# Zhangwenyao1/DreamVLA

Measured on AMD Instinct MI355X. Metric: train samples/sec (CALVIN ABC->D, seq_len=7), higher is better.
Workload: dtype bf16; 1 GPU; DreamVLA CALVIN finetune step, head set C (obs_pred+depth_pred+sam_feat_pred+use_dit_head), B=32/GPU, S=7, window 10, 2x224^2 views, 77 text tokens, hidden 1024 / 24 layers / 16 heads, dropout 0.1 on, AdamW + clip 0.1; global_batch=32, seq_len=7, parallelism=dp1, grad_exchange=GradBucketReducer (flat bf16 buckets, async all-reduce), optimizer=FlatAdamW (HIP: dvla_sumsq_bf16 + dvla_adamw_bf16 on flat buffers)

## Files before the change

### dreamvla_amd/csrc/attention.hip

```cpp
#include "common.h"
#include "launch.h"
#include "../../include/dvla.h"

namespace {

constexpr int AT_THREADS = 256;
constexpr int RM72 = 72;
constexpr int RM_BYTES = 32 * RM72 * 2;
constexpr int PI_BYTES = 16 * 64 * 4;
constexpr float LOG2E = 1.4426950408889634f;
constexpr float LN2 = 0.6931471805599453f;

struct AttnKArgs {
  const bf16_t *q, *k, *v; bf16_t* o;
  int64_t qsb, qst, qsh, ksb, kst, ksh, vsb, vst, vsh, osb, ost, osh;
  int B, H, Lq, Lk;
  float scale;
  const int32_t* key_index;
  const uint32_t *bits_q, *bits_k;
  const uint8_t* tile_map; int nqt, nkt;
  int has_drop; uint32_t drop_thr; float inv_keep; uint32_t seed_lo, seed_hi;
  float c1;
  float* lse;
  const bf16_t* dout; int64_t dsb, dst, dsh;
// ... 856 lines not shown
      const int qq = qt0 * 32 + ql;
      bits[i] = qq < p.Lq ? p.bits_q[(int64_t)qq * p.nkt + kt] : 0u;
    }
  uint32_t rowkey = 0;
  if (p.has_drop) rowkey = drop_rowkey(p.seed_lo, p.seed_hi, (uint32_t)rowid);
  f32x16 dqacc[2] = {zero16(), zero16()};
  __syncthreads();
  const TileWords tw = tile_words(flags, p.nkt, wave, lane);

  auto next_needed = [&](int kt) -> int {
    if (tw.n) return tw.next(kt);
    while (kt < p.nkt && __builtin_amdgcn_readfirstlane((int)flags[kt]) == 0) ++kt;
    return kt < p.nkt ? kt : -1;
  };
  const uint32_t smem_base = (uint32_t)(uintptr_t)(__attribute__((address_space(3))) char*)smem;
  const int rl = 8 * wave + (lane >> 3);
  const int oct = (lane & 7) ^ fa_sw(rl);
  const uint32_t kst2 = (uint32_t)p.kst * 2u, vst2 = (uint32_t)p.vst * 2u;
  auto issue = [&](int kt, int slot) {
    int row = kt * 32 + rl;
    row = row < p.Lk ? row : p.Lk - 1;
    const uint32_t src = p.key_index ? (uint32_t)kidx[row] : (uint32_t)row;
    const uint32_t dst = smem_base + (uint32_t)(slot * FA_STAGE + wave * 1024);
    fa_glds16(kb, src * kst2 + oct * 16, __builtin_amdgcn_readfirstlane(dst));
    fa_glds16(vb, src * vst2 + oct * 16, __builtin_amdgcn_readfirstlane(dst + FA_TILE));
  };

  int kt = next_needed(0);
  int kti = kt, islot = 0, cslot = 0, inflight = 0;
#pragma unroll
  for (int d = 0; d < FA_NS - 1; ++d)
    if (kti >= 0) {
      issue(kti, islot);
      islot = (islot + 1) & (FA_NS - 1); ++inflight;
      kti = next_needed(kti + 1);
    }
#pragma unroll
  for (int s = 0; s < 4; ++s) { fa_settle(qf[s]); fa_settle(dof[s]); }
  fa_settle(lse2); fa_settle(dlt);
  while (kt >= 0) {
    if (inflight >= 3) fa_wait_vmcnt<4>();
    else if (inflight == 2) fa_wait_vmcnt<2>();
    else fa_wait_vmcnt<0>();
    __builtin_amdgcn_s_barrier();
    __builtin_amdgcn_sched_barrier(0);
    --inflight;
    if (kti >= 0) {
      issue(kti, islot);
      islot = (islot + 1) & (FA_NS - 1); ++inflight;
      kti = next_needed(kti + 1);
    }
    __builtin_amdgcn_sched_barrier(0);
    const int flag = tw.n ? tw.flag(kt) : (__builtin_amdgcn_readfirstlane((int)flags[kt]) >> (2 * wave)) & 3;
    if (flag != 0) {
      const char* ks = smem + cslot * FA_STAGE;
      const char* vs = ks + FA_TILE;
      f32x16 sacc = zero16(), dpacc = zero16();
      {
        bf16x8 fk[4], fv[4];
#pragma unroll
        for (int s = 0; s < 4; ++s) { fk[s] = fa_frag_rm(ks, l31, s, g); fv[s] = fa_frag_rm(vs, l31, s, g); }
        fa_group4(fk); fa_group4(fv);
#pragma unroll
        for (int s = 0; s < 4; ++s) {
          sacc = __builtin_amdgcn_mfma_f32_32x32x16_bf16(fk[s], qf[s], sacc, 0, 0, 0);
          dpacc = __builtin_amdgcn_mfma_f32_32x32x16_bf16(fv[s], dof[s], dpacc, 0, 0, 0);
        }
      }
      const int k0 = kt * 32;
      uint32_t vis = 0xffffffffu;
      if (flag == 2) vis = bits[(wave * 32 + l31) * p.nkt + kt];
      if (k0 + 32 > p.Lk) vis &= low_mask(p.Lk - k0);
      float ds[16];
#pragma unroll
      for (int r = 0; r < 16; ++r) ds[r] = fast_exp2(fmaf(sacc[r], scale_log2, -lse2));
      if (__any(vis != 0xffffffffu)) {
        const uint32_t vg = vis >> (4 * g);
        vis_select16<0u>(vg, ds);
      }
      if (p.has_drop) {
        const uint32_t tk = drop_tilekey(rowkey, (uint32_t)kt);
        const uint32_t dx = drop_rot(tk, (uint32_t)g);
#pragma unroll
        for (int r = 0; r < 16; ++r) {
          const float dp = (drop_elem(dx, tk, DVLA_DROP_C(r)) >= p.drop_thr) ? dpacc[r] : 0.f;
          ds[r] = ds[r] * fmaf(dp, c1, -dlt);
        }
      } else {
#pragma unroll
        for (int r = 0; r < 16; ++r) ds[r] = ds[r] * fmaf(dpacc[r], c1, -dlt);
      }
      const bf16x8 f0 = pack_frag(ds), f1 = pack_frag(ds + 8);
      bf16x8 kt4[4];
#pragma unroll
      for (int i = 0; i < 4; ++i) kt4[i] = fa_frag_tr(ks, i >> 1, i & 1, lane);
      fa_group4(kt4);
      dqacc[0] = __builtin_amdgcn_mfma_f32_32x32x16_bf16(kt4[0], f0, dqacc[0], 0, 0, 0);
      dqacc[1] = __builtin_amdgcn_mfma_f32_32x32x16_bf16(kt4[2], f0, dqacc[1], 0, 0, 0);
      dqacc[0] = __builtin_amdgcn_mfma_f32_32x32x16_bf16(kt4[1], f1, dqacc[0], 0, 0, 0);
      dqacc[1] = __builtin_amdgcn_mfma_f32_32x32x16_bf16(kt4[3], f1, dqacc[1], 0, 0, 0);
    }
    __builtin_amdgcn_sched_barrier(0);
    cslot = (cslot + 1) & (FA_NS - 1);
    kt = next_needed(kt + 1);
  }
  if (q_ok) store_token(p.dq + (int64_t)b * p.dqsb + (int64_t)q * p.dqst + (int64_t)h * p.dqsh, dqacc, 1.0f, g, (p.st16 & 2) != 0);
}

__host__ __device__ inline size_t fa_dkv_smem_bytes(int nqt, bool has_bits, bool has_drop) {
  return (size_t)FA_RING + fa_pad16(nqt) + (has_bits ? (size_t)128 * nqt * 4 : 0) + (size_t)2 * 32 * nqt * 4 +
         (has_drop ? (size_t)4 * 32 * nqt * 4 : 0);
}

__global__ __launch_bounds__(AT_THREADS) void attn_bwd_dkv_ring_kernel(AttnKArgs p) {
  extern __shared__ __attribute__((aligned(16))) char smem[];
  const int t = threadIdx.x, lane = t & 63, l31 = lane & 31, g = lane >> 5;
  const int wave = __builtin_amdgcn_readfirstlane(t >> 6);
  const int b = blockIdx.z, h = blockIdx.y;
  const int kt0 = blockIdx.x * 4;
  const int ktw = kt0 + wave;
  const int key = ktw * 32 + l31;
  const bool key_ok = key < p.Lk;
  const int key_row = (key_ok && p.key_index) ? p.key_index[key] : key;
  const float scale_log2 = p.scale * LOG2E;
  const float c1 = p.c1;
  const bool has_bits = p.tile_map != nullptr && p.bits_k != nullptr;
  const bf16_t* qb = p.q + (int64_t)b * p.qsb + (int64_t)h * p.qsh;
  const bf16_t* kb = p.k + (int64_t)b * p.ksb + (int64_t)h * p.ksh;
  const bf16_t* vb = p.v + (int64_t)b * p.vsb + (int64_t)h * p.vsh;
  const bf16_t* dob = p.dout + (int64_t)b * p.dsb + (int64_t)h * p.dsh;
  const int bh_row0 = (b * p.H + h) * p.Lq;

  uint8_t* flags = reinterpret_cast<uint8_t*>(smem + FA_RING);
  uint32_t* bits = reinterpret_cast<uint32_t*>(smem + FA_RING + fa_pad16(p.nqt));
  float* lse2s = reinterpret_cast<float*>(smem + FA_RING + fa_pad16(p.nqt) + (has_bits ? (size_t)128 * p.nqt * 4 : 0));
  float* dlts = lse2s + 32 * p.nqt;
  uint32_t* tks = reinterpret_cast<uint32_t*>(dlts + 32 * p.nqt);

  bf16x8 kf[4], vf[4];
#pragma unroll
  for (int s = 0; s < 4; ++s) {
    const uint4 a = load16(kb + (int64_t)key_row * p.kst + 16 * s + 8 * g, key_ok);
    const uint4 c = load16(vb + (int64_t)key_row * p.vst + 16 * s + 8 * g, key_ok);
    kf[s] = *reinterpret_cast<const bf16x8*>(&a);
    vf[s] = *reinterpret_cast<const bf16x8*>(&c);
  }
  for (int qt = t; qt < p.nqt; qt += AT_THREADS) {
    int f = 0;
#pragma unroll
    for (int w = 0; w < 4; ++w) f |= tile_flag(p, qt, kt0 + w) << (2 * w);
    flags[qt] = (uint8_t)f;
  }
  if (has_bits)
    for (int i = t; i < 128 * p.nqt; i += AT_THREADS) {
      const int kl = i / p.nqt, qt = i - kl * p.nqt;
      const int kk = kt0 * 32 + kl;
      bits[i] = kk < p.Lk ? p.bits_k[(int64_t)kk * p.nqt + qt] : 0u;
    }
  for (int i = t; i < 32 * p.nqt; i += AT_THREADS) {
    lse2s[i] = i < p.Lq ? p.lse[bh_row0 + i] * LOG2E : INFINITY;
    dlts[i] = i < p.Lq ? p.delta[bh_row0 + i] * p.scale : 0.f;
    if (p.has_drop) {
      const uint32_t rk = drop_rowkey(p.seed_lo, p.seed_hi, (uint32_t)(bh_row0 + i));
#pragma unroll
      for (int w = 0; w < 4; ++w) tks[w * 32 * p.nqt + i] = drop_tilekey(rk, (uint32_t)(kt0 + w));
    }
  }
  const uint32_t drop_cj = DVLA_DROP_C((l31 & 3) + 4 * (l31 >> 3));
  const uint32_t drop_half = (uint32_t)((l31 >> 2) & 1);
  const uint32_t* tkw = tks + wave * 32 * p.nqt;
  f32x16 dkacc[2] = {zero16(), zero16()}, dvacc[2] = {zero16(), zero16()};
  __syncthreads();
  const TileWords tw = tile_words(flags, p.nqt, wave, lane);

  auto next_needed = [&](int qt) -> int {
    if (tw.n) return tw.next(qt);
    while (qt < p.nqt && __builtin_amdgcn_readfirstlane((int)flags[qt]) == 0) ++qt;
    return qt < p.nqt ? qt : -1;
  };
  const uint32_t smem_base = (uint32_t)(uintptr_t)(__attribute__((address_space(3))) char*)smem;
  const int rl = 8 * wave + (lane >> 3);
  const int oct = (lane & 7) ^ fa_sw(rl);
  const uint32_t qst2 = (uint32_t)p.qst * 2u, dst2 = (uint32_t)p.dst * 2u;
  auto issue = [&](int qt, int slot) {
    int row = qt * 32 + rl;
    row = row < p.Lq ? row : p.Lq - 1;
    const uint32_t dst = smem_base + (uint32_t)(slot * FA_STAGE + wave * 1024);
    fa_glds16(qb, (uint32_t)row * qst2 + oct * 16, __builtin_amdgcn_readfirstlane(dst));
    fa_glds16(dob, (uint32_t)row * dst2 + oct * 16, __builtin_amdgcn_readfirstlane(dst + FA_TILE));
  };

  int qt = next_needed(0);
  int qti = qt, islot = 0, cslot = 0, inflight = 0;
#pragma unroll
  for (int d = 0; d < FA_NS - 1; ++d)
    if (qti >= 0) {
      issue(qti, islot);
      islot = (islot + 1) & (FA_NS - 1); ++inflight;
      qti = next_needed(qti + 1);
    }
#pragma unroll
  for (int s = 0; s < 4; ++s) { fa_settle(kf[s]); fa_settle(vf[s]); }
  while (qt >= 0) {
    asm volatile("" : "+a"(dkacc[0]), "+a"(dkacc[1]), "+a"(dvacc[0]), "+a"(dvacc[1]));
    if (inflight >= 3) fa_wait_vmcnt<4>();
    else if (inflight == 2) fa_wait_vmcnt<2>();
    else fa_wait_vmcnt<0>();
    __builtin_amdgcn_s_barrier();
    __builtin_amdgcn_sched_barrier(0);
    --inflight;
    if (qti >= 0) {
      issue(qti, islot);
      islot = (islot + 1) & (FA_NS - 1); ++inflight;
      qti = next_needed(qti + 1);
    }
    __builtin_amdgcn_sched_barrier(0);
    const int flag = tw.n ? tw.flag(qt) : (__builtin_amdgcn_readfirstlane((int)flags[qt]) >> (2 * wave)) & 3;
    if (flag != 0) {
      const char* qs = smem + cslot * FA_STAGE;
      const char* dos = qs + FA_TILE;
      f32x16 sacc = zero16(), dpacc = zero16();
      {
        bf16x8 fq[4], fd[4];
#pragma unroll
        for (int s = 0; s < 4; ++s) { fq[s] = fa_frag_rm(qs, l31, s, g); fd[s] = fa_frag_rm(dos, l31, s, g); }
        fa_group4(fq); fa_group4(fd);
#pragma unroll
        for (int s = 0; s < 4; ++s) {
          sacc = __builtin_amdgcn_mfma_f32_32x32x16_bf16(fq[s], kf[s], sacc, 0, 0, 0);
          dpacc = __builtin_amdgcn_mfma_f32_32x32x16_bf16(fd[s], vf[s], dpacc, 0, 0, 0);
        }
      }
      asm volatile("" : "+v"(sacc), "+v"(dpacc));
      const int q0 = qt * 32;
      float lse2[16], dlt[16];
#pragma unroll
      for (int rq = 0; rq < 4; ++rq) {
        const float4 a = *reinterpret_cast<const float4*>(lse2s + q0 + 8 * rq + 4 * g);
        const float4 c = *reinterpret_cast<const float4*>(dlts + q0 + 8 * rq + 4 * g);
        lse2[4 * rq] = a.x; lse2[4 * rq + 1] = a.y; lse2[4 * rq + 2] = a.z; lse2[4 * rq + 3] = a.w;
        dlt[4 * rq] = c.x; dlt[4 * rq + 1] = c.y; dlt[4 * rq + 2] = c.z; dlt[4 * rq + 3] = c.w;
      }
      uint32_t vis = key_ok ? 0xffffffffu : 0u;
      if (flag == 2) vis = bits[(wave * 32 + l31) * p.nqt + qt];
      float pr[16], ds[16];
#pragma unroll
      for (int r = 0; r < 16; ++r) pr[r] = fast_exp2(fmaf(sacc[r], scale_log2, -lse2[r]));
      if (__any(vis != 0xffffffffu)) {
        const uint32_t vg = vis >> (4 * g);
        vis_select16<0u>(vg, pr);
      }
      float dp[16];
#pragma unroll
      for (int r = 0; r < 16; ++r) dp[r] = dpacc[r];
#pragma unroll
      for (int r = 0; r < 16; ++r) ds[r] = pr[r];
      if (p.has_drop) {
#pragma unroll
        for (int rq = 0; rq < 4; ++rq) {
          const uint4 a = *reinterpret_cast<const uint4*>(tkw + q0 + 8 * rq + 4 * g);
          const uint32_t rk[4] = {a.x, a.y, a.z, a.w};
#pragma unroll
          for (int e = 0; e < 4; ++e) {
            const int r = 4 * rq + e;
            const bool keep = drop_elem(drop_rot(rk[e], drop_half), rk[e], drop_cj) >= p.drop_thr;
            dp[r] = keep ? dp[r] : 0.f;
            pr[r] = keep ? pr[r] : 0.f;
          }
        }
      }
#pragma unroll
      for (int r = 0; r < 16; ++r) ds[r] = ds[r] * fmaf(dp[r], c1, -dlt[r]);
      const bf16x8 pf0 = pack_frag(pr), pf1 = pack_frag(pr + 8);
      const bf16x8 sf0 = pack_frag(ds), sf1 = pack_frag(ds + 8);
      {
        bf16x8 td[4], tq[4];
#pragma unroll
        for (int i = 0; i < 4; ++i) { td[i] = fa_frag_tr(dos, i >> 1, i & 1, lane); tq[i] = fa_frag_tr(qs, i >> 1, i & 1, lane); }
        fa_group4(td); fa_group4(tq);
        dvacc[0] = __builtin_amdgcn_mfma_f32_32x32x16_bf16(td[0], pf0, dvacc[0], 0, 0, 0);
        dkacc[0] = __builtin_amdgcn_mfma_f32_32x32x16_bf16(tq[0], sf0, dkacc[0], 0, 0, 0);
        dvacc[1] = __builtin_amdgcn_mfma_f32_32x32x16_bf16(td[2], pf0, dvacc[1], 0, 0, 0);
        dkacc[1] = __builtin_amdgcn_mfma_f32_32x32x16_bf16(tq[2], sf0, dkacc[1], 0, 0, 0);
        dvacc[0] = __builtin_amdgcn_mfma_f32_32x32x16_bf16(td[1], pf1, dvacc[0], 0, 0, 0);
        dkacc[0] = __builtin_amdgcn_mfma_f32_32x32x16_bf16(tq[1], sf1, dkacc[0], 0, 0, 0);
        dvacc[1] = __builtin_amdgcn_mfma_f32_32x32x16_bf16(td[3], pf1, dvacc[1], 0, 0, 0);
        dkacc[1] = __builtin_amdgcn_mfma_f32_32x32x16_bf16(tq[3], sf1, dkacc[1], 0, 0, 0);
      }
    }
    __builtin_amdgcn_sched_barrier(0);
    cslot = (cslot + 1) & (FA_NS - 1);
    qt = next_needed(qt + 1);
  }
  if (key_ok) {
    store_token(p.dk + (int64_t)b * p.dksb + (int64_t)key_row * p.dkst + (int64_t)h * p.dksh, dkacc, 1.0f, g, (p.st16 & 4) != 0);
    store_token(p.dv + (int64_t)b * p.dvsb + (int64_t)key_row * p.dvst + (int64_t)h * p.dvsh, dvacc, p.inv_keep, g, (p.st16 & 8) != 0);
  }
}


constexpr int SB_WAVES = 8, SB_THREADS = 64 * SB_WAVES, SB_MAX_TILES = 9;
__host__ __device__ inline size_t sb_smem_bytes(int nt) { return (size_t)nt * (4 * FA_TILE + 2 * 32 * 4); }

__global__ __launch_bounds__(SB_THREADS) void attn_bwd_short_kernel(AttnKArgs p) {
  extern __shared__ __attribute__((aligned(16))) char smem[];
  const int t = threadIdx.x, lane = t & 63, l31 = lane & 31, g = lane >> 5;
  const int wave = __builtin_amdgcn_readfirstlane(t >> 6);
  const int L = p.Lq;
  const int nt = p.nqt;
  const int rounds = (nt + SB_WAVES - 1) / SB_WAVES;
  const float scale_log2 = p.scale * LOG2E;

  char* const regA = smem;
  char* const regB = smem + (size_t)2 * nt * FA_TILE;
  float* const lse2s = reinterpret_cast<float*>(smem + (size_t)4 * nt * FA_TILE);
  float* const dlts = lse2s + 32 * nt;
  const uint32_t smem_base = (uint32_t)(uintptr_t)(__attribute__((address_space(3))) char*)smem;
  const uint32_t offA = 0u, offB = (uint32_t)(2 * nt * FA_TILE);

  const int rl = 8 * (wave & 3) + (lane >> 3);
  const int oct = (lane & 7) ^ fa_sw(rl);
  auto issue_op = [&](const bf16_t* base, uint32_t stride_bytes, uint32_t region) {
    for (int tt = wave >> 2; tt < nt; tt += 2) {
      int row = tt * 32 + rl;
      row = row < L ? row : L - 1;
      const uint32_t dst = smem_base + region + (uint32_t)(tt * FA_TILE + (wave & 3) * 1024);
      fa_glds16(base, (uint32_t)row * stride_bytes + (uint32_t)(oct * 16), __builtin_amdgcn_readfirstlane(dst));
    }
  };
  const uint32_t qst2 = (uint32_t)p.qst * 2u, kst2 = (uint32_t)p.kst * 2u, vst2 = (uint32_t)p.vst * 2u, dst2 = (uint32_t)p.dst * 2u;
  auto issue_A = [&](int item) {
    const int b = item / p.H, h = item - b * p.H;
    issue_op(p.q + (int64_t)b * p.qsb + (int64_t)h * p.qsh, qst2, offA);
    issue_op(p.dout + (int64_t)b * p.dsb + (int64_t)h * p.dsh, dst2, offA + (uint32_t)(nt * FA_TILE));
  };
  auto issue_A_tile = [&](int item, int tt) {
    const int b = item / p.H, h = item - b * p.H;
    int row = tt * 32 + rl;
    row = row < L ? row : L - 1;
    const uint32_t dst = smem_base + offA + (uint32_t)(tt * FA_TILE + (wave & 3) * 1024);
    fa_glds16(p.q + (int64_t)b * p.qsb + (int64_t)h * p.qsh, (uint32_t)row * qst2 + (uint32_t)(oct * 16), __builtin_amdgcn_readfirstlane(dst));
    fa_glds16(p.dout + (int64_t)b * p.dsb + (int64_t)h * p.dsh, (uint32_t)row * dst2 + (uint32_t)(oct * 16),
              __builtin_amdgcn_readfirstlane(dst + (uint32_t)(nt * FA_TILE)));
  };
  auto issue_B = [&](int item) {
    const int b = item / p.H, h = item - b * p.H;
    issue_op(p.k + (int64_t)b * p.ksb + (int64_t)h * p.ksh, kst2, offB);
    issue_op(p.v + (int64_t)b * p.vsb + (int64_t)h * p.vsh, vst2, offB + (uint32_t)(nt * FA_TILE));
  };

  const int n_items = p.B * p.H;
  int item = blockIdx.x;
  if (item >= n_items) return;
  issue_A(item);
  issue_B(item);

  uint4 ofr[4];
  float lse_in = 0.f;
  auto prefetch_o = [&](int it_) {
    const int b_ = it_ / p.H, h_ = it_ - b_ * p.H;
    const bf16_t* ob_ = p.o + (int64_t)b_ * p.osb + (int64_t)h_ * p.osh;
    const int q = wave * 32 + l31;
    const bool ok = wave < nt && q < L;
#pragma unroll
    for (int s = 0; s < 4; ++s) ofr[s] = load16(ob_ + (int64_t)q * p.ost + 16 * s + 8 * g, ok);
    lse_in = ok ? p.lse[(b_ * p.H + h_) * L + q] : 0.f;
  };
  prefetch_o(item);

  for (; item < n_items; item += gridDim.x) {
    const int b = item / p.H, h = item - b * p.H;
    const int next = item + (int)gridDim.x;
    const int row0 = (b * p.H + h) * L;
    const bf16_t* ob = p.o + (int64_t)b * p.osb + (int64_t)h * p.osh;

    fa_wait_vmcnt<0>();
#pragma unroll
    for (int s = 0; s < 4; ++s) { fa_settle(ofr[s].x); fa_settle(ofr[s].y); fa_settle(ofr[s].z); fa_settle(ofr[s].w); }
    fa_settle(lse_in);
    __syncthreads();

    for (int r = 0; r < rounds; ++r) {
      const int j = wave + SB_WAVES * r;
      if (j >= nt) break;
      const int q = j * 32 + l31;
      const bool q_ok = q < L;
      if (r > 0) {
#pragma unroll
        for (int s = 0; s < 4; ++s) ofr[s] = load16(ob + (int64_t)q * p.ost + 16 * s + 8 * g, q_ok);
        lse_in = q_ok ? p.lse[row0 + q] : 0.f;
      }
      const char* qs = regA + (size_t)j * FA_TILE;
      const char* dos = regA + (size_t)(nt + j) * FA_TILE;
      bf16x8 qf[4], dof[4];
#pragma unroll
      for (int s = 0; s < 4; ++s) { qf[s] = fa_frag_rm(qs, l31, s, g); dof[s] = fa_frag_rm(dos, l31, s, g); }
      float acc = 0.f;
#pragma unroll
      for (int s = 0; s < 4; ++s) {
        const uint4 dv = *reinterpret_cast<const uint4*>(&dof[s]);
        const uint32_t ow[4] = {ofr[s].x, ofr[s].y, ofr[s].z, ofr[s].w}, dw[4] = {dv.x, dv.y, dv.z, dv.w};
#pragma unroll
        for (int i = 0; i < 4; ++i) {
          acc += bf2f((bf16_t)(dw[i] & 0xffff)) * bf2f((bf16_t)(ow[i] & 0xffff));
          acc += bf2f((bf16_t)(dw[i] >> 16)) * bf2f((bf16_t)(ow[i] >> 16));
        }
      }
      acc += __shfl_xor(acc, 32, 64);
      const float lse2 = q_ok ? lse_in * LOG2E : INFINITY;
      const float dlt = q_ok ? acc * p.scale : 0.f;
      if (g == 0) { lse2s[j * 32 + l31] = lse2; dlts[j * 32 + l31] = dlt; }
      f32x16 dqacc[2] = {zero16(), zero16()};
      for (int kt = 0; kt < nt; ++kt) {
        const char* ks = regB + (size_t)kt * FA_TILE;
        const char* vs = regB + (size_t)(nt + kt) * FA_TILE;
        f32x16 sacc = zero16(), dpacc = zero16();
        {
          bf16x8 fk[4], fv[4];
#pragma unroll
          for (int s = 0; s < 4; ++s) { fk[s] = fa_frag_rm(ks, l31, s, g); fv[s] = fa_frag_rm(vs, l31, s, g); }
          fa_group4(fk); fa_group4(fv);
#pragma unroll
          for (int s = 0; s < 4; ++s) {
            sacc = __builtin_amdgcn_mfma_f32_32x32x16_bf16(fk[s], qf[s], sacc, 0, 0, 0);
            dpacc = __builtin_amdgcn_mfma_f32_32x32x16_bf16(fv[s], dof[s], dpacc, 0, 0, 0);
          }
        }
        const int k0 = kt * 32;
        float ds[16];
#pragma unroll
        for (int rr = 0; rr < 16; ++rr) ds[rr] = fast_exp2(fmaf(sacc[rr], scale_log2, -lse2));
        if (k0 + 32 > L) {
          asm volatile("");
          const uint32_t vg = low_mask(L - k0) >> (4 * g);
          vis_select16<0u>(vg, ds);
        }
#pragma unroll
        for (int rr = 0; rr < 16; ++rr) ds[rr] = ds[rr] * fmaf(dpacc[rr], p.scale, -dlt);
        const bf16x8 f0 = pack_frag(ds), f1 = pack_frag(ds + 8);
        bf16x8 kt4[4];
#pragma unroll
        for (int i = 0; i < 4; ++i) kt4[i] = fa_frag_tr(ks, i >> 1, i & 1, lane);
        fa_group4(kt4);
        dqacc[0] = __builtin_amdgcn_mfma_f32_32x32x16_bf16(kt4[0], f0, dqacc[0], 0, 0, 0);
        dqacc[1] = __builtin_amdgcn_mfma_f32_32x32x16_bf16(kt4[2], f0, dqacc[1], 0, 0, 0);
        dqacc[0] = __builtin_amdgcn_mfma_f32_32x32x16_bf16(kt4[1], f1, dqacc[0], 0, 0, 0);
        dqacc[1] = __builtin_amdgcn_mfma_f32_32x32x16_bf16(kt4[3], f1, dqacc[1], 0, 0, 0);
      }
      if (q_ok) store_token(p.dq + (int64_t)b * p.dqsb + (int64_t)q * p.dqst + (int64_t)h * p.dqsh, dqacc, 1.0f, g, (p.st16 & 2) != 0);
    }
    __syncthreads();

    for (int r = 0; r < rounds; ++r) {
      const int j = wave + SB_WAVES * r;
      const bool active = j < nt;
      const int key = j * 32 + l31;
      const bool key_ok = active && key < L;
      bf16x8 kf[4], vf[4];
      if (active) {
        const char* ks = regB + (size_t)j * FA_TILE;
        const char* vs = regB + (size_t)(nt + j) * FA_TILE;
#pragma unroll
        for (int s = 0; s < 4; ++s) { kf[s] = fa_frag_rm(ks, l31, s, g); vf[s] = fa_frag_rm(vs, l31, s, g); }
      }
      if (r == rounds - 1) {
        __syncthreads();
        if (next < n_items) { prefetch_o(next); issue_B(next); }
      }
      const bool last_round = r == rounds - 1;
      if (!active && !last_round) continue;
      f32x16 dkacc[2] = {zero16(), zero16()}, dvacc[2] = {zero16(), zero16()};
      for (int qt = 0; qt < nt; ++qt) {
        const char* qs = regA + (size_t)qt * FA_TILE;
        const char* dos = regA + (size_t)(nt + qt) * FA_TILE;
        if (qt > 0 && last_round) {
          __syncthreads();
          if (next < n_items && (wave >> 2) == ((qt - 1) & 1)) issue_A_tile(next, qt - 1);
        }
        if (!active) continue;
        f32x16 sacc = zero16(), dpacc = zero16();
        {
          bf16x8 fq[4], fd[4];
#pragma unroll
          for (int s = 0; s < 4; ++s) { fq[s] = fa_frag_rm(qs, l31, s, g); fd[s] = fa_frag_rm(dos, l31, s, g); }
          fa_group4(fq); fa_group4(fd);
#pragma unroll
          for (int s = 0; s < 4; ++s) {
            sacc = __builtin_amdgcn_mfma_f32_32x32x16_bf16(fq[s], kf[s], sacc, 0, 0, 0);
            dpacc = __builtin_amdgcn_mfma_f32_32x32x16_bf16(fd[s], vf[s], dpacc, 0, 0, 0);
          }
        }
        const int q0 = qt * 32;
        float pr[16], ds[16];
#pragma unroll
        for (int rq = 0; rq < 4; ++rq) {
          const float4 a = *reinterpret_cast<const float4*>(lse2s + q0 + 8 * rq + 4 * g);
          const float4 c = *reinterpret_cast<const float4*>(dlts + q0 + 8 * rq + 4 * g);
          const float l4[4] = {a.x, a.y, a.z, a.w}, d4[4] = {c.x, c.y, c.z, c.w};
#pragma unroll
          for (int e = 0; e < 4; ++e) {
            const int rr = 4 * rq + e;
            float pv = fast_exp2(fmaf(sacc[rr], scale_log2, -l4[e]));
            pv = key_ok ? pv : 0.f;
            pr[rr] = pv;
            ds[rr] = pv * fmaf(dpacc[rr], p.scale, -d4[e]);
          }
        }
        const bf16x8 pf0 = pack_frag(pr), pf1 = pack_frag(pr + 8);
        const bf16x8 sf0 = pack_frag(ds), sf1 = pack_frag(ds + 8);
        {
          bf16x8 td[4], tq[4];
#pragma unroll
          for (int i = 0; i < 4; ++i) { td[i] = fa_frag_tr(dos, i >> 1, i & 1, lane); tq[i] = fa_frag_tr(qs, i >> 1, i & 1, lane); }
          fa_group4(td); fa_group4(tq);
          dvacc[0] = __builtin_amdgcn_mfma_f32_32x32x16_bf16(td[0], pf0, dvacc[0], 0, 0, 0);
          dkacc[0] = __builtin_amdgcn_mfma_f32_32x32x16_bf16(tq[0], sf0, dkacc[0], 0, 0, 0);
          dvacc[1] = __builtin_amdgcn_mfma_f32_32x32x16_bf16(td[2], pf0, dvacc[1], 0, 0, 0);
          dkacc[1] = __builtin_amdgcn_mfma_f32_32x32x16_bf16(tq[2], sf0, dkacc[1], 0, 0, 0);
          dvacc[0] = __builtin_amdgcn_mfma_f32_32x32x16_bf16(td[1], pf1, dvacc[0], 0, 0, 0);
          dkacc[0] = __builtin_amdgcn_mfma_f32_32x32x16_bf16(tq[1], sf1, dkacc[0], 0, 0, 0);
          dvacc[1] = __builtin_amdgcn_mfma_f32_32x32x16_bf16(td[3], pf1, dvacc[1], 0, 0, 0);
          dkacc[1] = __builtin_amdgcn_mfma_f32_32x32x16_bf16(tq[3], sf1, dkacc[1], 0, 0, 0);
        }
      }
      if (key_ok) {
        store_token(p.dk + (int64_t)b * p.dksb + (int64_t)key * p.dkst + (int64_t)h * p.dksh, dkacc, 1.0f, g, (p.st16 & 4) != 0);
        store_token(p.dv + (int64_t)b * p.dvsb + (int64_t)key * p.dvst + (int64_t)h * p.dvsh, dvacc, 1.0f, g, (p.st16 & 8) != 0);
      }
    }
    __syncthreads();
    if (next < n_items && (wave >> 2) == ((nt - 1) & 1)) issue_A_tile(next, nt - 1);
  }
}


__host__ __device__ inline size_t sf_smem_bytes(int nt) { return (size_t)nt * 2 * FA_TILE; }

__global__ __launch_bounds__(SB_THREADS) __attribute__((amdgpu_waves_per_eu(4, 4))) void attn_fwd_short_kernel(AttnKArgs p) {
  extern __shared__ __attribute__((aligned(16))) char smem[];
  const int t = threadIdx.x, lane = t & 63, l31 = lane & 31, g = lane >> 5;
  const int wave = __builtin_amdgcn_readfirstlane(t >> 6);
  const int L = p.Lq;
  const int nt = p.nqt;
  const int rounds = (nt + SB_WAVES - 1) / SB_WAVES;
  const float scale_log2 = p.scale * LOG2E;
  const uint32_t smem_base = (uint32_t)(uintptr_t)(__attribute__((address_space(3))) char*)smem;
  const int rl = 8 * (wave & 3) + (lane >> 3);
  const int oct = (lane & 7) ^ fa_sw(rl);
  const uint32_t kst2 = (uint32_t)p.kst * 2u, vst2 = (uint32_t)p.vst * 2u;
  auto issue_op = [&](const bf16_t* base, uint32_t stride_bytes, uint32_t region) {
    for (int tt = wave >> 2; tt < nt; tt += 2) {
      int row = tt * 32 + rl;
      row = row < L ? row : L - 1;
      const uint32_t dst = smem_base + region + (uint32_t)(tt * FA_TILE + (wave & 3) * 1024);
      fa_glds16(base, (uint32_t)row * stride_bytes + (uint32_t)(oct * 16), __builtin_amdgcn_readfirstlane(dst));
    }
  };
  const int n_items = p.B * p.H;
  for (int item = blockIdx.x; item < n_items; item += gridDim.x) {
    const int b = item / p.H, h = item - b * p.H;
    const bf16_t* qb = p.q + (int64_t)b * p.qsb + (int64_t)h * p.qsh;
    issue_op(p.k + (int64_t)b * p.ksb + (int64_t)h * p.ksh, kst2, 0u);
    issue_op(p.v + (int64_t)b * p.vsb + (int64_t)h * p.vsh, vst2, (uint32_t)(nt * FA_TILE));
    for (int r = 0; r < rounds; ++r) {
      const int j = wave + SB_WAVES * r;
      const bool active = j < nt;
      const int q = j * 32 + l31;
      const bool q_ok = active && q < L;
      bf16x8 qf[4];
#pragma unroll
      for (int s = 0; s < 4; ++s) {
        const uint4 u = load16(qb + (int64_t)q * p.qst + 16 * s + 8 * g, q_ok);
        qf[s] = *reinterpret_cast<const bf16x8*>(&u);
      }
      if (r == 0) {
        fa_wait_vmcnt<0>();
        __syncthreads();
      }
      if (!active) continue;
      float m_run = -INFINITY, l_run = 0.f;
      f32x16 oacc[2] = {zero16(), zero16()};
      for (int kt = 0; kt < nt; ++kt) {
        const char* ks = smem + (size_t)kt * FA_TILE;
        const char* vs = smem + (size_t)(nt + kt) * FA_TILE;
        f32x16 sacc = zero16();
        {
          bf16x8 fk[4];
#pragma unroll
          for (int s = 0; s < 4; ++s) fk[s] = fa_frag_rm(ks, l31, s, g);
          fa_group4(fk);
#pragma unroll
          for (int s = 0; s < 4; ++s) sacc = __builtin_amdgcn_mfma_f32_32x32x16_bf16(fk[s], qf[s], sacc, 0, 0, 0);
        }
        const int k0 = kt * 32;
        float sv[16];
#pragma unroll
        for (int rr = 0; rr < 16; ++rr) sv[rr] = sacc[rr];
        if (k0 + 32 > L) {
          asm volatile("");
          const uint32_t vg = low_mask(L - k0) >> (4 * g);
          vis_select16<NEG_INF_BITS>(vg, sv);
        }
        float mt = sv[0];
#pragma unroll
        for (int rr = 1; rr < 16; ++rr) mt = fmaxf(mt, sv[rr]);
        mt = fmaxf(mt, __shfl_xor(mt, 32, 64));
        const float m_new = fmaxf(m_run, ceilf(mt * scale_log2));
        const float m_safe = (m_new == -INFINITY) ? 0.f : m_new;
        const float alpha = fast_exp2(m_run - m_safe);
        float rs = 0.f;
#pragma unroll
        for (int rr = 0; rr < 16; ++rr) { sv[rr] = fast_exp2(fmaf(sv[rr], scale_log2, -m_safe)); rs += sv[rr]; }
        rs += __shfl_xor(rs, 32, 64);
        l_run = l_run * alpha + rs;
        m_run = m_new;
        if (__any(alpha != 1.0f)) {
#pragma unroll
          for (int rr = 0; rr < 16; ++rr) { oacc[0][rr] *= alpha; oacc[1][rr] *= alpha; }
        }
        bf16x8 vt4[4];
#pragma unroll
        for (int i = 0; i < 4; ++i) vt4[i] = fa_frag_tr(vs, i >> 1, i & 1, lane);
        __builtin_amdgcn_sched_barrier(0);
        const bf16x8 pf0 = pack_frag(sv), pf1 = pack_frag(sv + 8);
        fa_group4(vt4);
        oacc[0] = __builtin_amdgcn_mfma_f32_32x32x16_bf16(vt4[0], pf0, oacc[0], 0, 0, 0);
        oacc[1] = __builtin_amdgcn_mfma_f32_32x32x16_bf16(vt4[2], pf0, oacc[1], 0, 0, 0);
        oacc[0] = __builtin_amdgcn_mfma_f32_32x32x16_bf16(vt4[1], pf1, oacc[0], 0, 0, 0);
        oacc[1] = __builtin_amdgcn_mfma_f32_32x32x16_bf16(vt4[3], pf1, oacc[1], 0, 0, 0);
      }
      if (q_ok) {
        const float inv_l = l_run > 0.f ? 1.0f / l_run : 0.f;
        store_token(p.o + (int64_t)b * p.osb + (int64_t)q * p.ost + (int64_t)h * p.osh, oacc, inv_l, g, (p.st16 & 1) != 0);
        if (p.lse && g == 0) p.lse[(b * p.H + h) * L + q] = l_run > 0.f ? (m_run + log2f(l_run)) * LN2 : INFINITY;
      }
    }
    __syncthreads();
  }
}


}

static bool attn_span32(int64_t rows, int64_t stride_elems, bool gathered) {
  const int64_t r = gathered ? (rows > (1 << 18) ? rows : (1 << 18)) : rows;
  return stride_elems >= 0 && r * stride_elems * 2 + 128 < (1LL << 32);
}

static bool attn_force_staged() {
  static int v = -1;
  if (v < 0) { const char* e = getenv("DVLA_ATTN_STAGED"); v = (e && e[0] == '1') ? 1 : 0; }
  return v == 1;
}

static bool attn_short_enabled() { const char* e = getenv("DVLA_ATTN_SHORT"); return !(e && e[0] == '0'); }
static bool attn_short_fwd_enabled() { const char* e = getenv("DVLA_ATTN_SHORT_FWD"); return !(e && e[0] == '0'); }
static int attn_num_cus() { const int n = dvla_num_cus(); return n > 0 ? n : 256; }

#ifdef DVLA_ATTN_ABLATION
static int attn_dbg() { const char* e = getenv("DVLA_ATTN_DBG"); return e ? atoi(e) : 0; }
#endif

static dim3 ring_items_grid(int nblk, const AttnKArgs& a) {
  static int forced = -1;
  if (forced < 0) { const char* e = getenv("DVLA_ATTN_ITEMS"); forced = e ? atoi(e) : 0; }
  const int cus = attn_num_cus();
  const int nqb = nblk, items = a.B * a.H;
  int y = items;
  const bool tables = a.tile_map != nullptr || a.key_index != nullptr;
  if (forced > 0) y = (items + forced - 1) / forced;
  else if (tables) { const int by4 = (items + 3) / 4, fill = (3 * cus + nqb - 1) / nqb; y = by4 > fill ? by4 : fill; if (y > items) y = items; }
  if (y < 1) y = 1;
  if (y > 65535) y = 65535;
  return dim3((unsigned)nqb, (unsigned)y, 1u);
}
static dim3 fwd_ring_grid(const AttnKArgs& a) { return ring_items_grid((a.nqt + 3) / 4, a); }

extern "C" int dvla_attn_fwd(const dvla_attn_params* q, void* stream_) {
  hipStream_t stream = reinterpret_cast<hipStream_t>(stream_);
  AttnKArgs a;
  int rc = fill_args(q, a);
  if (rc != DVLA_OK) return rc;
  dim3 grid((unsigned)((a.nqt + 3) / 4), (unsigned)a.H, (unsigned)a.B), block(AT_THREADS);
  const dim3 ring_grid = fwd_ring_grid(a);
  const size_t smem = fa_smem_bytes(a.nkt, a.Lk, a.key_index != nullptr, a.tile_map != nullptr && a.bits_q != nullptr);
  const bool span_kv = attn_span32(a.Lk, a.kst, a.key_index != nullptr) && attn_span32(a.Lk, a.vst, a.key_index != nullptr);
  if (attn_short_fwd_enabled() && !a.tile_map && !a.key_index && !a.has_drop && a.Lq == a.Lk && a.nqt > 2 && a.nqt <= SB_MAX_TILES &&
      span_kv && !attn_force_staged()) {
    const size_t sm = sf_smem_bytes(a.nqt);
    (void)dvla_allow_lds(attn_fwd_short_kernel, 80 * 1024);
    const int64_t items = (int64_t)a.B * a.H;
    int64_t wgs = (int64_t)attn_num_cus() * 2;
    if (wgs > items) wgs = items;
    hipLaunchKernelGGL(attn_fwd_short_kernel, dim3((unsigned)wgs), dim3(SB_THREADS), sm, stream, a);
    return dvla_check_launch();
  }
  if (smem <= 64 * 1024 && span_kv && !attn_force_staged())
#ifndef DVLA_ATTN_ABLATION
    hipLaunchKernelGGL(attn_fwd_ring_kernel<0>, ring_grid, block, smem, stream, a);
#else
    switch (attn_dbg()) {
      case 1: hipLaunchKernelGGL(attn_fwd_ring_kernel<1>, ring_grid, block, smem, stream, a); break;
      case 2: hipLaunchKernelGGL(attn_fwd_ring_kernel<2>, ring_grid, block, smem, stream, a); break;
      case 4: hipLaunchKernelGGL(attn_fwd_ring_kernel<4>, ring_grid, block, smem, stream, a); break;
      case 8: hipLaunchKernelGGL(attn_fwd_ring_kernel<8>, ring_grid, block, smem, stream, a); break;
      case 16: hipLaunchKernelGGL(attn_fwd_ring_kernel<16>, ring_grid, block, smem, stream, a); break;
      case 14: hipLaunchKernelGGL(attn_fwd_ring_kernel<14>, ring_grid, block, smem, stream, a); break;
      case 15: hipLaunchKernelGGL(attn_fwd_ring_kernel<15>, ring_grid, block, smem, stream, a); break;
      case 31: hipLaunchKernelGGL(attn_fwd_ring_kernel<31>, ring_grid, block, smem, stream, a); break;
      case 63: hipLaunchKernelGGL(attn_fwd_ring_kernel<63>, ring_grid, block, smem, stream, a); break;
      case 64: hipLaunchKernelGGL(attn_fwd_ring_kernel<64>, ring_grid, block, smem, stream, a); break;
      default: hipLaunchKernelGGL(attn_fwd_ring_kernel<0>, ring_grid, block, smem, stream, a); break;
    }
#endif
  else
    hipLaunchKernelGGL(attn_fwd_kernel, grid, block, 0, stream, a);
  return dvla_check_launch();
}

extern "C" int dvla_attn_bwd(const dvla_attn_params* q, void* stream_) {
  hipStream_t stream = reinterpret_cast<hipStream_t>(stream_);
  AttnKArgs a;
  int rc = fill_args(q, a);
  if (rc != DVLA_OK) return rc;
  if (!q->dout || !q->lse || !q->delta || !q->dq || !q->dk || !q->dv) return DVLA_ERR_ARG;
  if (q->tile_map && !q->mask_bits_k) return DVLA_ERR_ARG;
  if (!dvla_aligned(q->dout, q->do_stride_b, q->do_stride_t, q->do_stride_h, 16)) return DVLA_ERR_UNSUPPORTED;
  if (!dvla_aligned(q->dq, q->dq_stride_b, q->dq_stride_t, q->dq_stride_h, 8) || !dvla_aligned(q->dk, q->dk_stride_b, q->dk_stride_t, q->dk_stride_h, 8) ||
      !dvla_aligned(q->dv, q->dv_stride_b, q->dv_stride_t, q->dv_stride_h, 8) || !dvla_aligned(q->o, q->o_stride_b, q->o_stride_t, q->o_stride_h, 16))
    return DVLA_ERR_UNSUPPORTED;
  const int64_t nrows = (int64_t)a.B * a.H * a.Lq;
  dim3 block(AT_THREADS);
  const bool span_all = attn_span32(a.Lk, a.kst, false) && attn_span32(a.Lk, a.vst, false) && attn_span32(a.Lq, a.qst, false) &&
                        attn_span32(a.Lq, a.dst, false);
  if (attn_short_enabled() && !a.tile_map && !a.key_index && !a.has_drop && a.Lq == a.Lk && a.nqt <= SB_MAX_TILES && span_all &&
      !attn_force_staged()) {
    const size_t smem = sb_smem_bytes(a.nqt);
    (void)dvla_allow_lds(attn_bwd_short_kernel, 160 * 1024);
    int per_cu = (int)((size_t)(160 * 1024) / smem);
    if (per_cu < 1) per_cu = 1;
    if (per_cu > 2048 / SB_THREADS) per_cu = 2048 / SB_THREADS;
    const int64_t items = (int64_t)a.B * a.H;
    int64_t wgs = (int64_t)attn_num_cus() * per_cu;
    if (wgs > items) wgs = items;
    hipLaunchKernelGGL(attn_bwd_short_kernel, dim3((unsigned)wgs), dim3(SB_THREADS), smem, stream, a);
    return dvla_check_launch();
  }
  const size_t smem_dq = fa_smem_bytes(a.nkt, a.Lk, a.key_index != nullptr, a.tile_map != nullptr && a.bits_q != nullptr);
  const size_t smem_dkv = fa_dkv_smem_bytes(a.nqt, a.tile_map != nullptr && a.bits_k != nullptr, a.has_drop != 0);
  const dim3 grid_dq((unsigned)((a.nqt + 3) / 4), (unsigned)a.H, (unsigned)a.B);
  const dim3 grid_dkv((unsigned)((a.nkt + 3) / 4), (unsigned)a.H, (unsigned)a.B);
  const bool span_kv = attn_span32(a.Lk, a.kst, a.key_index != nullptr) && attn_span32(a.Lk, a.vst, a.key_index != nullptr);
  const bool span_q = attn_span32(a.Lq, a.qst, false) && attn_span32(a.Lq, a.dst, false);
  const bool dq_ring = smem_dq <= 64 * 1024 && span_kv && !attn_force_staged();
  a.fuse_delta = dq_ring ? 1 : 0;
  if (!dq_ring) {
    hipLaunchKernelGGL(attn_delta_kernel, dim3((unsigned)((nrows * 8 + 255) / 256)), dim3(256), 0, stream, a);
    rc = dvla_check_launch();
    if (rc != DVLA_OK) return rc;
  }
  if (dq_ring)
    hipLaunchKernelGGL(attn_bwd_dq_ring_kernel, grid_dq, block, smem_dq, stream, a);
  else
    hipLaunchKernelGGL(attn_bwd_dq_kernel, grid_dq, block, 0, stream, a);
  rc = dvla_check_launch();
  if (rc != DVLA_OK) return rc;
  if (smem_dkv <= 80 * 1024 && span_q && !attn_force_staged()) {
    if (smem_dkv > 64 * 1024) (void)dvla_allow_lds(attn_bwd_dkv_ring_kernel, 80 * 1024);
    hipLaunchKernelGGL(attn_bwd_dkv_ring_kernel, grid_dkv, block, smem_dkv, stream, a);
  }
  else
    hipLaunchKernelGGL(attn_bwd_dkv_kernel, grid_dkv, block, 0, stream, a);
  return dvla_check_launch();
}
```

Baseline: 238.5 samples/s.

## Software-pipeline short-sequence attention backward: prefetch next tile's QK/dP MFMAs during softmax

```diff
diff --git a/dreamvla_amd/csrc/attention.hip b/dreamvla_amd/csrc/attention.hip
--- a/dreamvla_amd/csrc/attention.hip
+++ b/dreamvla_amd/csrc/attention.hip
@@ -1182,6 +1182,36 @@
 constexpr int SB_WAVES = 8, SB_THREADS = 64 * SB_WAVES, SB_MAX_TILES = 9;
 __host__ __device__ inline size_t sb_smem_bytes(int nt) { return (size_t)nt * (4 * FA_TILE + 2 * 32 * 4); }
 
+__device__ __forceinline__ uint32_t sf_ofs_rm(int l31, int g) { return (uint32_t)(l31 * 128 + ((g ^ fa_sw(l31)) << 4)); }
+__device__ __forceinline__ uint32_t sf_ofs_tr(int lane) {
+  const int r0 = 4 * (lane >> 5) + ((lane & 15) >> 2), d0 = 16 * ((lane >> 4) & 1) + 4 * (lane & 3);
+  return (uint32_t)(r0 * 128 + (((d0 >> 3) ^ fa_sw(r0)) << 4) + (d0 & 7) * 2);
+}
+__device__ __forceinline__ uint32_t sf_tile_addr(uint32_t ofs, int tile) {
+  uint32_t a = ofs + (uint32_t)tile * FA_TILE;
+  asm("" : "+v"(a));
+  return a;
+}
+__device__ __forceinline__ void sf_pin8(float* x) {
+  asm volatile("" : "+v"(x[0]), "+v"(x[1]), "+v"(x[2]), "+v"(x[3]), "+v"(x[4]), "+v"(x[5]), "+v"(x[6]), "+v"(x[7]));
+}
+__device__ __forceinline__ void sf_pin4(uint32_t& a, uint32_t& b, uint32_t& c, uint32_t& d) { asm volatile("" : "+v"(a), "+v"(b), "+v"(c), "+v"(d)); }
+__device__ __forceinline__ void sf_read_rm4(bf16x8 (&f)[4], const char* base, uint32_t a) {
+#pragma unroll
+  for (int s = 0; s < 4; ++s) f[s] = *reinterpret_cast<const bf16x8*>(base + (a ^ (uint32_t)(s << 5)));
+}
+__device__ __forceinline__ void sf_read_tr4(bf16x8 (&f)[4], const char* base, uint32_t a) {
+#pragma unroll
+  for (int i = 0; i < 4; ++i) {
+    union { fa_s16x4 h[2]; bf16x8 v; } u;
+#pragma unroll
+    for (int h = 0; h < 2; ++h)
+      u.h[h] = __builtin_amdgcn_ds_read_tr16_b64_v4i16((__attribute__((address_space(3))) fa_s16x4*)(
+          base + (a ^ (uint32_t)(((i >> 1) << 6) | (h << 5))) + (i & 1) * 2048 + h * 1024));
+    f[i] = u.v;
+  }
+}
+
 __global__ __launch_bounds__(SB_THREADS) void attn_bwd_short_kernel(AttnKArgs p) {
   extern __shared__ __attribute__((aligned(16))) char smem[];
   const int t = threadIdx.x, lane = t & 63, l31 = lane & 31, g = lane >> 5;
@@ -1190,6 +1220,7 @@
   const int nt = p.nqt;
   const int rounds = (nt + SB_WAVES - 1) / SB_WAVES;
   const float scale_log2 = p.scale * LOG2E;
+  const uint32_t ofs_rm = sf_ofs_rm(l31, g), ofs_tr = sf_ofs_tr(lane);
 
   char* const regA = smem;
   char* const regB = smem + (size_t)2 * nt * FA_TILE;
@@ -1216,7 +1247,9 @@
   };
   auto issue_A_tile = [&](int item, int tt) {
     const int b = item / p.H, h = item - b * p.H;
-    int row = tt * 32 + rl;
+    int rl_ = rl;
+    asm volatile("" : "+v"(rl_));
+    int row = tt * 32 + rl_;
     row = row < L ? row : L - 1;
     const uint32_t dst = smem_base + offA + (uint32_t)(tt * FA_TILE + (wave & 3) * 1024);
     fa_glds16(p.q + (int64_t)b * p.qsb + (int64_t)h * p.qsh, (uint32_t)row * qst2 + (uint32_t)(oct * 16), __builtin_amdgcn_readfirstlane(dst));
@@ -1237,10 +1270,11 @@
 
   uint4 ofr[4];
   float lse_in = 0.f;
+  auto row_of_lane = [&]() __attribute__((always_inline)) { int r_ = l31; asm volatile("" : "+v"(r_)); return r_; };
   auto prefetch_o = [&](int it_) {
     const int b_ = it_ / p.H, h_ = it_ - b_ * p.H;
     const bf16_t* ob_ = p.o + (int64_t)b_ * p.osb + (int64_t)h_ * p.osh;
-    const int q = wave * 32 + l31;
+    const int q = wave * 32 + row_of_lane();
     const bool ok = wave < nt && q < L;
 #pragma unroll
     for (int s = 0; s < 4; ++s) ofr[s] = load16(ob_ + (int64_t)q * p.ost + 16 * s + 8 * g, ok);
@@ -1263,7 +1297,7 @@
     for (int r = 0; r < rounds; ++r) {
       const int j = wave + SB_WAVES * r;
       if (j >= nt) break;
-      const int q = j * 32 + l31;
+      const int q = j * 32 + row_of_lane();
       const bool q_ok = q < L;
       if (r > 0) {
 #pragma unroll
@@ -1291,42 +1325,85 @@
       const float dlt = q_ok ? acc * p.scale : 0.f;
       if (g == 0) { lse2s[j * 32 + l31] = lse2; dlts[j * 32 + l31] = dlt; }
       f32x16 dqacc[2] = {zero16(), zero16()};
-      for (int kt = 0; kt < nt; ++kt) {
-        const char* ks = regB + (size_t)kt * FA_TILE;
-        const char* vs = regB + (size_t)(nt + kt) * FA_TILE;
-        f32x16 sacc = zero16(), dpacc = zero16();
-        {
-          bf16x8 fk[4], fv[4];
-#pragma unroll
-          for (int s = 0; s < 4; ++s) { fk[s] = fa_frag_rm(ks, l31, s, g); fv[s] = fa_frag_rm(vs, l31, s, g); }
-          fa_group4(fk); fa_group4(fv);
-#pragma unroll
-          for (int s = 0; s < 4; ++s) {
-            sacc = __builtin_amdgcn_mfma_f32_32x32x16_bf16(fk[s], qf[s], sacc, 0, 0, 0);
-            dpacc = __builtin_amdgcn_mfma_f32_32x32x16_bf16(fv[s], dof[s], dpacc, 0, 0, 0);
-          }
-        }
+      auto read_kv = [&](bf16x8 (&fk)[4], bf16x8 (&fv)[4], int kt) __attribute__((always_inline)) {
+        const uint32_t a = sf_tile_addr(ofs_rm, 2 * nt + kt);
+        sf_read_rm4(fk, smem, a);
+        sf_read_rm4(fv, smem, a + (uint32_t)nt * FA_TILE);
+      };
+      auto tile_x = [&](const f32x16& sacc, const f32x16& dpacc, f32x16& sn, f32x16& dpn, int kt, bool ahead, bool maybe_last)
+                        __attribute__((always_inline)) {
+        bf16x8 fk[4], fv[4];
+        if (ahead) { read_kv(fk, fv, kt + 1); __builtin_amdgcn_sched_barrier(0); }
         const int k0 = kt * 32;
         float ds[16];
 #pragma unroll
-        for (int rr = 0; rr < 16; ++rr) ds[rr] = fast_exp2(fmaf(sacc[rr], scale_log2, -lse2));
-        if (k0 + 32 > L) {
+        for (int rr = 0; rr < 8; ++rr) ds[rr] = fast_exp2(fmaf(sacc[rr], scale_log2, -lse2));
+        if (ahead) {
+          sf_pin8(ds);
+          __builtin_amdgcn_sched_barrier(0);
+          fa_group4(fk); fa_group4(fv);
+          sn = __builtin_amdgcn_mfma_f32_32x32x16_bf16(fk[0], qf[0], zero16(), 0, 0, 0);
+          dpn = __builtin_amdgcn_mfma_f32_32x32x16_bf16(fv[0], dof[0], zero16(), 0, 0, 0);
+          sn = __builtin_amdgcn_mfma_f32_32x32x16_bf16(fk[1], qf[1], sn, 0, 0, 0);
+          dpn = __builtin_amdgcn_mfma_f32_32x32x16_bf16(fv[1], dof[1], dpn, 0, 0, 0);
+          __builtin_amdgcn_sched_barrier(0);
+        }
+#pragma unroll
+        for (int rr = 8; rr < 16; ++rr) ds[rr] = fast_exp2(fmaf(sacc[rr], scale_log2, -lse2));
+        if (maybe_last && k0 + 32 > L) {
           asm volatile("");
           const uint32_t vg = low_mask(L - k0) >> (4 * g);
           vis_select16<0u>(vg, ds);
         }
+        if (ahead) {
+          sf_pin8(ds + 8);
+          __builtin_amdgcn_sched_barrier(0);
+          sn = __builtin_amdgcn_mfma_f32_32x32x16_bf16(fk[2], qf[2], sn, 0, 0, 0);
+          dpn = __builtin_amdgcn_mfma_f32_32x32x16_bf16(fv[2], dof[2], dpn, 0, 0, 0);
+          __builtin_amdgcn_sched_barrier(0);
+        }
 #pragma unroll
         for (int rr = 0; rr < 16; ++rr) ds[rr] = ds[rr] * fmaf(dpacc[rr], p.scale, -dlt);
+        if (ahead) {
+          sf_pin8(ds); sf_pin8(ds + 8);
+          __builtin_amdgcn_sched_barrier(0);
+          sn = __builtin_amdgcn_mfma_f32_32x32x16_bf16(fk[3], qf[3], sn, 0, 0, 0);
+          dpn = __builtin_amdgcn_mfma_f32_32x32x16_bf16(fv[3], dof[3], dpn, 0, 0, 0);
+          __builtin_amdgcn_sched_barrier(0);
+        }
         const bf16x8 f0 = pack_frag(ds), f1 = pack_frag(ds + 8);
         bf16x8 kt4[4];
-#pragma unroll
-        for (int i = 0; i < 4; ++i) kt4[i] = fa_frag_tr(ks, i >> 1, i & 1, lane);
+        sf_read_tr4(kt4, smem, sf_tile_addr(ofs_tr, 2 * nt + kt));
         fa_group4(kt4);
         dqacc[0] = __builtin_amdgcn_mfma_f32_32x32x16_bf16(kt4[0], f0, dqacc[0], 0, 0, 0);
         dqacc[1] = __builtin_amdgcn_mfma_f32_32x32x16_bf16(kt4[2], f0, dqacc[1], 0, 0, 0);
         dqacc[0] = __builtin_amdgcn_mfma_f32_32x32x16_bf16(kt4[1], f1, dqacc[0], 0, 0, 0);
         dqacc[1] = __builtin_amdgcn_mfma_f32_32x32x16_bf16(kt4[3], f1, dqacc[1], 0, 0, 0);
-      }
+        __builtin_amdgcn_sched_barrier(0);
+      };
+      f32x16 sa = zero16(), dpa = zero16(), sb, dpb;
+      {
+        bf16x8 fk[4], fv[4];
+        read_kv(fk, fv, 0);
+        fa_group4(fk); fa_group4(fv);
+#pragma unroll
+        for (int s = 0; s < 4; ++s) {
+          sa = __builtin_amdgcn_mfma_f32_32x32x16_bf16(fk[s], qf[s], sa, 0, 0, 0);
+          dpa = __builtin_amdgcn_mfma_f32_32x32x16_bf16(fv[s], dof[s], dpa, 0, 0, 0);
+        }
+      }
+      __builtin_amdgcn_sched_barrier(0);
+      int kt = 0;
+      for (; kt + 2 < nt; kt += 2) {
+        tile_x(sa, dpa, sb, dpb, kt, true, false);
+        tile_x(sb, dpb, sa, dpa, kt + 1, true, false);
+      }
+      if (kt + 1 < nt) {
+        tile_x(sa, dpa, sb, dpb, kt, true, false);
+        sa = sb; dpa = dpb;
+        ++kt;
+      }
+      tile_x(sa, dpa, sb, dpb, kt, false, true);
       if (q_ok) store_token(p.dq + (int64_t)b * p.dqsb + (int64_t)q * p.dqst + (int64_t)h * p.dqsh, dqacc, 1.0f, g, (p.st16 & 2) != 0);
     }
     __syncthreads();
@@ -1334,7 +1411,7 @@
     for (int r = 0; r < rounds; ++r) {
       const int j = wave + SB_WAVES * r;
       const bool active = j < nt;
-      const int key = j * 32 + l31;
+      const int key = j * 32 + row_of_lane();
       const bool key_ok = active && key < L;
       bf16x8 kf[4], vf[4];
       if (active) {
@@ -1350,58 +1427,99 @@
       const bool last_round = r == rounds - 1;
       if (!active && !last_round) continue;
       f32x16 dkacc[2] = {zero16(), zero16()}, dvacc[2] = {zero16(), zero16()};
-      for (int qt = 0; qt < nt; ++qt) {
-        const char* qs = regA + (size_t)qt * FA_TILE;
-        const char* dos = regA + (size_t)(nt + qt) * FA_TILE;
+      auto walk_sync = [&](int qt) __attribute__((always_inline)) {
         if (qt > 0 && last_round) {
           __syncthreads();
           if (next < n_items && (wave >> 2) == ((qt - 1) & 1)) issue_A_tile(next, qt - 1);
         }
-        if (!active) continue;
-        f32x16 sacc = zero16(), dpacc = zero16();
+      };
+      if (!active) {
+        for (int qt = 0; qt < nt; ++qt) walk_sync(qt);
+      } else {
+        auto read_qd = [&](bf16x8 (&fq)[4], bf16x8 (&fd)[4], int qt) __attribute__((always_inline)) {
+          const uint32_t a = sf_tile_addr(ofs_rm, qt);
+          sf_read_rm4(fq, smem, a);
+          sf_read_rm4(fd, smem, a + (uint32_t)nt * FA_TILE);
+        };
+        auto tile_y = [&](const f32x16& sacc, const f32x16& dpacc, f32x16& sn, f32x16& dpn, int qt, bool ahead)
+                          __attribute__((always_inline)) {
+          bf16x8 fq[4], fd[4];
+          if (ahead) { read_qd(fq, fd, qt + 1); __builtin_amdgcn_sched_barrier(0); }
+          const int q0 = qt * 32;
+          union { uint32_t w[4]; bf16x8 v; } pf[2], sf[2];
+#pragma unroll
+          for (int rq = 0; rq < 4; ++rq) {
+            const float4 a = *reinterpret_cast<const float4*>(lse2s + q0 + 8 * rq + 4 * g);
+            const float4 c = *reinterpret_cast<const float4*>(dlts + q0 + 8 * rq + 4 * g);
+            const float l4[4] = {a.x, a.y, a.z, a.w}, d4[4] = {c.x, c.y, c.z, c.w};
+            float pr[4], ds[4];
+#pragma unroll
+            for (int e = 0; e < 4; ++e) {
+              const int rr = 4 * rq + e;
+              float pv = fast_exp2(fmaf(sacc[rr], scale_log2, -l4[e]));
+              pv = key_ok ? pv : 0.f;
+              pr[e] = pv;
+              ds[e] = pv * fmaf(dpacc[rr], p.scale, -d4[e]);
+            }
+            pf[rq >> 1].w[2 * (rq & 1)] = pack2bf(pr[0], pr[1]); pf[rq >> 1].w[2 * (rq & 1) + 1] = pack2bf(pr[2], pr[3]);
+            sf[rq >> 1].w[2 * (rq & 1)] = pack2bf(ds[0], ds[1]); sf[rq >> 1].w[2 * (rq & 1) + 1] = pack2bf(ds[2], ds[3]);
+            if (ahead && (rq == 1 || rq == 2)) {
+              sf_pin4(pf[rq >> 1].w[2 * (rq & 1)], pf[rq >> 1].w[2 * (rq & 1) + 1], sf[rq >> 1].w[2 * (rq & 1)], sf[rq >> 1].w[2 * (rq & 1) + 1]);
+              __builtin_amdgcn_sched_barrier(0);
+              if (rq == 1) { fa_group4(fq); fa_group4(fd); }
+              const int s0 = 2 * (rq - 1);
+              sn = __builtin_amdgcn_mfma_f32_32x32x16_bf16(fq[s0], kf[s0], rq == 1 ? zero16() : sn, 0, 0, 0);
+              dpn = __builtin_amdgcn_mfma_f32_32x32x16_bf16(fd[s0], vf[s0], rq == 1 ? zero16() : dpn, 0, 0, 0);
+              sn = __builtin_amdgcn_mfma_f32_32x32x16_bf16(fq[s0 + 1], kf[s0 + 1], sn, 0, 0, 0);
+              dpn = __builtin_amdgcn_mfma_f32_32x32x16_bf16(fd[s0 + 1], vf[s0 + 1], dpn, 0, 0, 0);
+              __builtin_amdgcn_sched_barrier(0);
+            }
+          }
+          const bf16x8 pf0 = pf[0].v, pf1 = pf[1].v, sf0 = sf[0].v, sf1 = sf[1].v;
+          {
+            bf16x8 td[4], tq[4];
+            const uint32_t a = sf_tile_addr(ofs_tr, qt);
+            sf_read_tr4(tq, smem, a);
+            sf_read_tr4(td, smem, a + (uint32_t)nt * FA_TILE);
+            fa_group4(td); fa_group4(tq);
+            dvacc[0] = __builtin_amdgcn_mfma_f32_32x32x16_bf16(td[0], pf0, dvacc[0], 0, 0, 0);
+            dkacc[0] = __builtin_amdgcn_mfma_f32_32x32x16_bf16(tq[0], sf0, dkacc[0], 0, 0, 0);
+            dvacc[1] = __builtin_amdgcn_mfma_f32_32x32x16_bf16(td[2], pf0, dvacc[1], 0, 0, 0);
+            dkacc[1] = __builtin_amdgcn_mfma_f32_32x32x16_bf16(tq[2], sf0, dkacc[1], 0, 0, 0);
+            dvacc[0] = __builtin_amdgcn_mfma_f32_32x32x16_bf16(td[1], pf1, dvacc[0], 0, 0, 0);
+            dkacc[0] = __builtin_amdgcn_mfma_f32_32x32x16_bf16(tq[1], sf1, dkacc[0], 0, 0, 0);
+            dvacc[1] = __builtin_amdgcn_mfma_f32_32x32x16_bf16(td[3], pf1, dvacc[1], 0, 0, 0);
+            dkacc[1] = __builtin_amdgcn_mfma_f32_32x32x16_bf16(tq[3], sf1, dkacc[1], 0, 0, 0);
+          }
+          __builtin_amdgcn_sched_barrier(0);
+        };
+        f32x16 sa = zero16(), dpa = zero16(), sb, dpb;
         {
           bf16x8 fq[4], fd[4];
-#pragma unroll
-          for (int s = 0; s < 4; ++s) { fq[s] = fa_frag_rm(qs, l31, s, g); fd[s] = fa_frag_rm(dos, l31, s, g); }
+          read_qd(fq, fd, 0);
           fa_group4(fq); fa_group4(fd);
 #pragma unroll
           for (int s = 0; s < 4; ++s) {
-            sacc = __builtin_amdgcn_mfma_f32_32x32x16_bf16(fq[s], kf[s], sacc, 0, 0, 0);
-            dpacc = __builtin_amdgcn_mfma_f32_32x32x16_bf16(fd[s], vf[s], dpacc, 0, 0, 0);
+            sa = __builtin_amdgcn_mfma_f32_32x32x16_bf16(fq[s], kf[s], sa, 0, 0, 0);
+            dpa = __builtin_amdgcn_mfma_f32_32x32x16_bf16(fd[s], vf[s], dpa, 0, 0, 0);
           }
         }
-        const int q0 = qt * 32;
-        float pr[16], ds[16];
-#pragma unroll
-        for (int rq = 0; rq < 4; ++rq) {
-          const float4 a = *reinterpret_cast<const float4*>(lse2s + q0 + 8 * rq + 4 * g);
-          const float4 c = *reinterpret_cast<const float4*>(dlts + q0 + 8 * rq + 4 * g);
-          const float l4[4] = {a.x, a.y, a.z, a.w}, d4[4] = {c.x, c.y, c.z, c.w};
-#pragma unroll
-          for (int e = 0; e < 4; ++e) {
-            const int rr = 4 * rq + e;
-            float pv = fast_exp2(fmaf(sacc[rr], scale_log2, -l4[e]));
-            pv = key_ok ? pv : 0.f;
-            pr[rr] = pv;
-            ds[rr] = pv * fmaf(dpacc[rr], p.scale, -d4[e]);
-          }
+        __builtin_amdgcn_sched_barrier(0);
+        int qt = 0;
+        for (; qt + 2 < nt; qt += 2) {
+          walk_sync(qt);
+          tile_y(sa, dpa, sb, dpb, qt, true);
+          walk_sync(qt + 1);
+          tile_y(sb, dpb, sa, dpa, qt + 1, true);
         }
-        const bf16x8 pf0 = pack_frag(pr), pf1 = pack_frag(pr + 8);
-        const bf16x8 sf0 = pack_frag(ds), sf1 = pack_frag(ds + 8);
-        {
-          bf16x8 td[4], tq[4];
-#pragma unroll
-          for (int i = 0; i < 4; ++i) { td[i] = fa_frag_tr(dos, i >> 1, i & 1, lane); tq[i] = fa_frag_tr(qs, i >> 1, i & 1, lane); }
-          fa_group4(td); fa_group4(tq);
-          dvacc[0] = __builtin_amdgcn_mfma_f32_32x32x16_bf16(td[0], pf0, dvacc[0], 0, 0, 0);
-          dkacc[0] = __builtin_amdgcn_mfma_f32_32x32x16_bf16(tq[0], sf0, dkacc[0], 0, 0, 0);
-          dvacc[1] = __builtin_amdgcn_mfma_f32_32x32x16_bf16(td[2], pf0, dvacc[1], 0, 0, 0);
-          dkacc[1] = __builtin_amdgcn_mfma_f32_32x32x16_bf16(tq[2], sf0, dkacc[1], 0, 0, 0);
-          dvacc[0] = __builtin_amdgcn_mfma_f32_32x32x16_bf16(td[1], pf1, dvacc[0], 0, 0, 0);
-          dkacc[0] = __builtin_amdgcn_mfma_f32_32x32x16_bf16(tq[1], sf1, dkacc[0], 0, 0, 0);
-          dvacc[1] = __builtin_amdgcn_mfma_f32_32x32x16_bf16(td[3], pf1, dvacc[1], 0, 0, 0);
-          dkacc[1] = __builtin_amdgcn_mfma_f32_32x32x16_bf16(tq[3], sf1, dkacc[1], 0, 0, 0);
+        if (qt + 1 < nt) {
+          walk_sync(qt);
+          tile_y(sa, dpa, sb, dpb, qt, true);
+          sa = sb; dpa = dpb;
+          ++qt;
         }
+        walk_sync(qt);
+        tile_y(sa, dpa, sb, dpb, qt, false);
       }
       if (key_ok) {
         store_token(p.dk + (int64_t)b * p.dksb + (int64_t)key * p.dkst + (int64_t)h * p.dksh, dkacc, 1.0f, g, (p.st16 & 4) != 0);
```

New measurement: 238.5 samples/s. No clear change (-0.0%).
